# mnhrk15/integrated_path_planning

Measured on AMD Instinct MI355X. Metric: candidate trajectories/sec, higher is better.
Workload: dtype f64; 1 GPU; config4: 256 ego instances/GPU x 2240-candidate lattice (5 s, dt 0.1 s), 20-sample x 30-pedestrian x 51-step fp32 prediction distribution (layout [S][P][T][2]), eps=0; 8 distinct batches rotated (501 MB of obstacle tensors per GPU); instances_per_gpu=256, instances_total=256, rotation_batches=8, plan_calls_in_flight=4

## Files before the change

### integrated_path_planning_amd/csrc/fot_kernels.hip

```cpp
#include <hip/hip_runtime.h>

#include <cstdlib>
#include <cstring>

#include "fot_math.hpp"
#include "fot_kernels.h"

namespace fot {


template <int CTRL, int ROW_MASK>
__device__ __forceinline__ float dpp_f32(float v)
{
    return __int_as_float(__builtin_amdgcn_update_dpp(__float_as_int(v), __float_as_int(v), CTRL, ROW_MASK, 0xf, false));
}

#define FOT_WAVE_REDUCE_F32(NAME, OP)                                                        \
    __device__ __forceinline__ float NAME(float v)                                           \
    {                                                                                        \
        v = OP(v, dpp_f32<0xB1, 0xf>(v));                           \
        v = OP(v, dpp_f32<0x4E, 0xf>(v));                           \
        v = OP(v, dpp_f32<0x141, 0xf>(v));                              \
        v = OP(v, dpp_f32<0x140, 0xf>(v));                                   \
        v = OP(v, dpp_f32<0x142, 0xa>(v));                     \
// ... 376 lines not shown
    if ((int)blockIdx.x < n_inst) {
        if (mixed) {
            const int scen = (imp.h_desc ? imp.h_desc : desc)[blockIdx.x].scen;
            Pp += scen;
            sp_hbm = load_const(sp_table, scen);
        }
        sp = stage_spline(sp_hbm, lds_knots);
    }
    frenet_state_block(Pp, sp, desc, state, n_inst, imp, scan, inst_done, (int)blockIdx.x, gh, all_waves);
}


__device__ __forceinline__ double uniform_f64(double v)
{
    int lo = __builtin_amdgcn_readfirstlane(__double2loint(v));
    int hi = __builtin_amdgcn_readfirstlane(__double2hiint(v));
    asm volatile("" : "+s"(lo), "+s"(hi));
    return __hiloint2double(hi, lo);
}

typedef float f16 __attribute__((ext_vector_type(16)));

template <int OFF>
__device__ __forceinline__ void sload_chunk(f16 &dst, const f2x8 *src)
{
    asm volatile("s_load_dwordx16 %0, %1, %2" : "=s"(dst) : "s"(src), "n"(OFF) : "memory");
}

template <int OFF>
__device__ __forceinline__ void sload_chunk_ahead(f16 &dst, const f2x8 *src, float &ahead)
{
    asm volatile("s_load_dwordx16 %0, %2, %3" : "=s"(dst), "+v"(ahead) : "s"(src), "n"(OFF) : "memory");
}

__device__ __forceinline__ void swait_chunk(f16 &c)
{
    asm volatile("s_waitcnt lgkmcnt(0)" : "+s"(c) : : "memory");
}

typedef float v2f __attribute__((ext_vector_type(2)));

__device__ __forceinline__ float min_sqdist32_f16(const f16 &c, float fx, float fy)
{
    const v2f px = { fx, fx }, py = { fy, fy };
    v2f t[ENT_CHUNK / 2];
#pragma unroll
    for (int j = 0; j < ENT_CHUNK / 2; ++j) {
        const v2f ox = { c[2 * j], c[2 * j + 1] }, oy = { c[8 + 2 * j], c[8 + 2 * j + 1] };
        const v2f dx = px - ox, dy = py - oy;
        t[j] = __builtin_elementwise_fma(dy, dy, dx * dx);
    }
    float m = fminf(fminf(t[0].x, t[0].y), t[1].x);
    m = fminf(fminf(m, t[1].y), t[2].x);
    m = fminf(fminf(m, t[2].y), t[3].x);
    return fminf(m, t[3].y);
}

__device__ __forceinline__ float min_sqdist32_walk(const f2x8 *cp, int n, float &fx, float fy)
{
    float m = INFINITY;
    f16 ca, cb;
    sload_chunk<0>(ca, cp);
    swait_chunk(ca);
    for (int c = 0; c < n; c += 2) {
        sload_chunk_ahead<64>(cb, cp, fx);
        m = fminf(m, min_sqdist32_f16(ca, fx, fy));
        swait_chunk(cb);
        sload_chunk_ahead<128>(ca, cp, fx);
        if (c + 1 < n) m = fminf(m, min_sqdist32_f16(cb, fx, fy));
        swait_chunk(ca);
        cp += 2;
    }
    return m;
}

template <typename T>
__device__ __forceinline__ void st_agent(T *p, T v) { __hip_atomic_store(p, v, __ATOMIC_RELAXED, __HIP_MEMORY_SCOPE_AGENT); }
template <typename T>
__device__ __forceinline__ T ld_agent(const T *p) { return __hip_atomic_load(p, __ATOMIC_RELAXED, __HIP_MEMORY_SCOPE_AGENT); }

struct EvalKernArgs {
    const DevParams *Pp; SplineView sp; const InstDesc *desc; const InstState *state;
    int row_budget, lds_knots, ablate, n_inst, max_tiles;
    const SplineView *sp_table; int mixed;
    const int32_t *tile_cand0;
    const GroupHead *heads;
    const TileStep *wave_rng; const f2 *ent32; const d2 *ent64; const uint8_t *ent_sid;
    double *cand_cost; uint8_t *cand_status; uint16_t *cand_keep;
    TilePart *parts;
    fot_result *out; int32_t *inst_done;
    int32_t *done_flag; int32_t done_seq;
};
constexpr int EVAL_LEAD_PTRS = 7;
__device__ __forceinline__ const EvalKernArgs &eval_kernargs()
{
    return *(const EvalKernArgs *)((const char *)__builtin_amdgcn_kernarg_segment_ptr() + EVAL_LEAD_PTRS * sizeof(void *));
}

template <bool LEAN>
struct FusedSink {
    const DevParams *Pp;
    const InstDesc *Dp;
    uint32_t my_rng;
    float my_thr, my_thr_sure;
    float my_thr_fatal;
    int step_base;
    int step_row;
    int lane_id;
    float thr, thr_fatal;
    const f2x8 *chunks;
    int chunks_per_k;
    uint64_t hit_mask;
    int viol;
    bool hit;
    int c_lo, n_chunks;
    uint32_t pf;
    bool no_warm;

    __device__ __forceinline__ void steps_load(int base)
    {
        const DevParams &P = *Pp;
        const EvalKernArgs &KA = eval_kernargs();
        TileStep st = { 0u, 0.0f, 0.0f, 0u };
        if (Dp->ent_cap != 0 && base + lane_id < P.n_total && !(KA.ablate & 1))
            st = KA.wave_rng[(int64_t)step_row * P.n_total + base + lane_id];
        my_rng = st.rng; my_thr = st.thr; my_thr_sure = st.thr_sure;
        my_thr_fatal = Dp->max_viol == 0 ? st.thr_sure : -1.0f;
        step_base = base;
    }

    __device__ __forceinline__ void row_begin(int k)
    {
        if constexpr (!LEAN)
            if ((k & ~(WAVE - 1)) != step_base) steps_load(k & ~(WAVE - 1));
        const int kl = LEAN ? k : k & (WAVE - 1);
        const uint32_t r = (uint32_t)__builtin_amdgcn_readlane((int)my_rng, kl);
        c_lo = (int)(r >> 16);
        n_chunks = (int)(r & 0xffffu) - c_lo;
        thr = __builtin_bit_cast(float, __builtin_amdgcn_readlane(__builtin_bit_cast(int, my_thr), kl));
        thr_fatal = __builtin_bit_cast(float, __builtin_amdgcn_readlane(__builtin_bit_cast(int, LEAN ? my_thr_sure : my_thr_fatal), kl));
        if (n_chunks > 0 && !no_warm) {
            const f2x8 *row = chunks + (int64_t)k * chunks_per_k + c_lo;
            asm volatile("s_load_dword %0, %1, 0x0\n\t"
                         "s_load_dword %0, %1, 0x40\n\t"
                         "s_load_dword %0, %1, 0x80\n\t"
                         "s_load_dword %0, %1, 0xc0"
                         : "=&s"(pf) : "s"(row) : "memory");
        } else {
            pf = 0;
        }
    }

    __device__ __forceinline__ void row_end(int) { asm volatile("s_waitcnt lgkmcnt(0)" : "+s"(pf) : : "memory"); }

    __device__ __forceinline__ void put(int k, int ci, double px, double py, bool alive)
    {
        put32(k, ci, (float)px, (float)py, alive, [&](double &ex, double &ey) { ex = px; ey = py; });
    }

    template <class GetExact>
    __device__ __forceinline__ void put32(int k, int, float fx_in, float fy, bool alive, const GetExact &get_exact)
    {
        if (n_chunks == 0) return;
        if (!alive || hit) return;
        float fx = fx_in;
        const f2x8 *row = chunks + (int64_t)k * chunks_per_k + c_lo;
        if (LEAN || thr_fatal >= 0.0f) {
            const float m = min_sqdist32_walk(row, n_chunks, fx, fy);
            if (m <= thr_fatal) { hit = true; return; }
            if (!(m <= thr)) return;
        }
        bool sure = false;
        for (int c0 = 0; c0 < n_chunks; c0 += 32) {
            const int nb = n_chunks - c0 < 32 ? n_chunks - c0 : 32;
            const f2x8 *cp = row + c0;
            uint32_t near_bits = 0;
            f16 ca, cb;
            sload_chunk<0>(ca, cp);
            swait_chunk(ca);
            for (int c = 0; c < nb; c += 2) {
                sload_chunk_ahead<64>(cb, cp, fx);
                const float ma = min_sqdist32_f16(ca, fx, fy);
                near_bits = (near_bits << 1) | (uint32_t)(ma <= thr);
                sure |= ma <= thr_fatal;
                swait_chunk(cb);
                sload_chunk_ahead<128>(ca, cp, fx);
                if (c + 1 < nb) {
                    const float mb = min_sqdist32_f16(cb, fx, fy);
                    near_bits = (near_bits << 1) | (uint32_t)(mb <= thr);
                    sure |= mb <= thr_fatal;
                }
                swait_chunk(ca);
                cp += 2;
            }
            if (sure) { hit = true; return; }
            if (near_bits != 0) {
                double px, py;
                get_exact(px, py);
                exact(k, c0, nb, near_bits, px, py, fx, fy);
            }
        }
    }

    __device__ __forceinline__ void exact(int k, int c0, int nb, uint32_t near_bits, double px, double py, float fx,
                                          float fy)
    {
        const DevParams &P = *Pp;
        const InstDesc &D = *Dp;
        px += D.ego.x; py += D.ego.y;
        const double sq_dyn = D.dyn_mode == FOT_DYN_SINGLE ? P.sq_r_dyn : P.sq_r;
        const EvalKernArgs &KA = eval_kernargs();
        const float thr_sure = LEAN ? thr_fatal :
            __builtin_bit_cast(float, __builtin_amdgcn_readlane(__builtin_bit_cast(int, my_thr_sure), k & (WAVE - 1)));
        const d2 *e64 = KA.ent64 + D.ent_off;
        const uint8_t *sid = KA.ent_sid + D.ent_off;
        const int64_t base = ((int64_t)k * chunks_per_k + c_lo) * ENT_CHUNK;
        uint64_t mask_l = 0;
        int viol_l = 0;
        while (near_bits != 0 && !hit) {
            const int hb = 31 - __clz((int)near_bits);
            near_bits &= ~(1u << hb);
            const int64_t e = base + (int64_t)(c0 + nb - 1 - hb) * ENT_CHUNK;
            if constexpr (LEAN)
                exact_chunk_f32first(chunks[e / ENT_CHUNK], e64 + e, sid + e, fx, fy, thr, thr_sure, px, py, P.sq_r, sq_dyn,
                                     0, mask_l, viol_l, hit);
            else
                exact_chunk_f32first(chunks[e / ENT_CHUNK], e64 + e, sid + e, fx, fy, thr, thr_sure, px, py, P.sq_r, sq_dyn,
                                     D.max_viol, hit_mask, viol, hit);
        }
    }

    __device__ __forceinline__ bool collided() const { return hit; }
};

constexpr int EVAL_WG = WAVES_PER_GROUP * WAVE;
extern __shared__ double s_lon[];

constexpr int ROW_FIELDS = 9;
constexpr int LONINFO_DOUBLES = (int)(sizeof(LonInfo) / sizeof(double));
static_assert(sizeof(LonInfo) % sizeof(double) == 0, "LonInfo sits in the double-typed LDS array");
__host__ __device__ constexpr int eval_wave_doubles(int row_budget)
{
    return row_budget * ROW_FIELDS + TILE_MAX_PROFILES * LONINFO_DOUBLES + TILE_MAX_PROFILES / 2;
}
__host__ __device__ constexpr int eval_group_doubles()
{
    return GROUP_ROWS * ROW_FIELDS + (int)(sizeof(GroupHead) / sizeof(double));
}
constexpr int SEG_MAX = 4;
constexpr int SEG_F64 = 4, SEG_I32 = 4;
constexpr int SEG_DOUBLES = (SEG_F64 + SEG_I32 / 2) * WAVE;

struct StagedTab {
    static constexpr bool LOCAL = true;
    int lds_row0;
    int k_max;
    double dt;
#ifdef FOT_TIMELINE
    mutable uint64_t t_rows = 0;
#endif
    __device__ __forceinline__ void load(int k, LonSample &L) const
    {
#ifdef FOT_TIMELINE
        const uint64_t t0 = __builtin_amdgcn_s_memtime();
#endif
        const int kk = k < k_max ? k : k_max;
        const double *r = s_lon + lds_row0 + kk * ROW_FIELDS;
        L.s = 0.0; L.sd = r[0]; L.sdd = r[1]; L.rx = r[2]; L.ry = r[3];
        L.cos_r = r[4]; L.sin_r = r[5]; L.kr = r[6]; L.dkr = r[7]; L.inv_sd = r[8];
        asm volatile("" : "+v"(L.sd), "+v"(L.sdd), "+v"(L.rx), "+v"(L.ry), "+v"(L.cos_r), "+v"(L.sin_r),
                          "+v"(L.kr), "+v"(L.dkr), "+v"(L.inv_sd));
#ifdef FOT_TIMELINE
        t_rows += __builtin_amdgcn_s_memtime() - t0;
#endif
    }
    const LonInfo *info;
    __device__ __forceinline__ double s_at(int k) const
    {
        double s_, u0, u1, u2;
        lon_sample(*info, k, dt, s_, u0, u1, u2);
        return s_;
    }
};

#ifdef FOT_TIMELINE
__device__ uint64_t g_timeline[4 * 16384];
__device__ uint64_t g_shader_clock[2 * 16384];
__device__ uint64_t g_row_wait[16384];
__device__ uint64_t g_phase[4 * 16384];
__shared__ uint64_t s_tl_entry[2];
extern "C" int fot_timeline_read_phase(uint64_t *out, int n_words)
{
    return (int)hipMemcpyFromSymbol(out, HIP_SYMBOL(g_phase), sizeof(uint64_t) * (size_t)n_words);
}
extern "C" int fot_timeline_read_rows(uint64_t *out, int n_words)
{
    return (int)hipMemcpyFromSymbol(out, HIP_SYMBOL(g_row_wait), sizeof(uint64_t) * (size_t)n_words);
}
extern "C" int fot_timeline_read(uint64_t *out, int n_words)
{
    return (int)hipMemcpyFromSymbol(out, HIP_SYMBOL(g_timeline), sizeof(uint64_t) * (size_t)n_words);
}
extern "C" int fot_timeline_read_clock(uint64_t *out, int n_words)
{
    return (int)hipMemcpyFromSymbol(out, HIP_SYMBOL(g_shader_clock), sizeof(uint64_t) * (size_t)n_words);
}
#endif

__device__ __forceinline__ void wave_lds_fence()
{
    __builtin_amdgcn_fence(__ATOMIC_SEQ_CST, "wavefront");
    __builtin_amdgcn_wave_barrier();
}

__device__ __forceinline__ void tile_results(const DevParams &P, const InstDesc &D, const StagedTab &tab, const LonInfo &L,
                                             const double *q, SegState &g, bool hit, bool has_cand, int64_t slot, int cand0,
                                             int lane, TilePart &tp)
{
    int st_final = FOT_ST_DROPPED;
    ScanBest mine = { INFINITY, -1 };
    int my_keep = 0;
    if (has_cand) {
        CandResult r;
        {
            LonInfo Lf = *tab.info;
            Lf.n_t = L.n_t;
            finish_candidate(P, D, Lf, tab, q, g, hit, r);
        }
        st_final = final_status(r.status, r.v_last, r.travel, D.max_stop);
        const EvalKernArgs &KA = eval_kernargs();
        KA.cand_cost[slot] = r.cost;
        KA.cand_status[slot] = (uint8_t)st_final;
        KA.cand_keep[slot] = (uint16_t)r.keep;
        my_keep = r.keep;
        mine = select_entry(st_final, r.cost, cand0 + lane);
    }
    {
        const ScanBest best = wave_argmin(mine);
        tp.cost = best.dist; tp.idx = best.idx;
        tp.keep = __builtin_amdgcn_readfirstlane(__shfl(my_keep, best.idx >= 0 ? best.idx - cand0 : 0, WAVE));
#pragma unroll
        for (int c = 0; c < 8; ++c) tp.cnt[c] = __popcll(__ballot(st_final == c));
    }
}

enum { TILE_WAVE = 0, TILE_SPLIT = 1 };
template <int MODE, bool LEAN>
__device__ __forceinline__ void evaluate_tile(const DevParams *__restrict__ Pp, const InstDesc *__restrict__ desc,
                                              const InstState *__restrict__ state,
                                              const int32_t *__restrict__ tile_cand0, const int32_t *__restrict__ tile_n,
                                              const TileStep *__restrict__ wave_rng, const f2 *__restrict__ ent32,
                                              const EvalKernArgs &a, const SplineView &sp_lds,
                                              double *my_rows, int inst, int tile, int lane, int tl_tag, TilePart &tp,
                                              int sub = 0, int n_sub = 1, double *s_part = nullptr)
{
    constexpr bool SPLIT = MODE == TILE_SPLIT;
    const int seg = SPLIT ? sub : 0, n_seg = SPLIT ? n_sub : 1;
    const DevParams &P = *Pp;
    const InstDesc &D = desc[inst];
    const InstState &S = state[inst];
    const int n_total = P.n_total;
    const int cand0 = tile_cand0[D.shape_off + tile];
    int n = tile_n[D.shape_off + tile];
    int stage_c0 = cand0, stage_c1 = cand0 + n;
    if (n <= 0) return;
    if (!S.c2f_ok || stage_c0 >= S.n_cand) return;
    if (stage_c1 > S.n_cand) stage_c1 = S.n_cand;
    if (cand0 + n > S.n_cand) n = S.n_cand - cand0 > 0 ? S.n_cand - cand0 : 0;
#ifdef FOT_TIMELINE
    const uint64_t t_blk = __builtin_amdgcn_s_memrealtime();
#endif
    LonInfo *s_info = (LonInfo *)(my_rows + a.row_budget * ROW_FIELDS);
    int *s_row0 = (int *)(s_info + TILE_MAX_PROFILES);
    const int slot_lo = decode_candidate(P, D, S.frenet0, stage_c0).lon_slot;
    const int n_stage = decode_candidate(P, D, S.frenet0, stage_c1 - 1).lon_slot - slot_lo + 1;
    const auto lds_fence = [] { if constexpr (MODE != TILE_WAVE) __syncthreads(); else wave_lds_fence(); };
    if constexpr (MODE == TILE_WAVE) wave_lds_fence();
    const int bld_id = (MODE == TILE_WAVE ? 0 : sub * WAVE) + lane, bld_n = (MODE == TILE_WAVE ? 1 : n_sub) * WAVE;
    int total_rows = 0, n_loop = 0;
    for (int p = 0; p < n_stage; ++p) {
        const int r = profile_rows(P, D, slot_lo + p);
        if (bld_id == p) s_row0[p] = total_rows;
        total_rows += r;
    }
    if (bld_id < n_stage) s_info[bld_id] = profile_info(P, D, S.frenet0, slot_lo + bld_id, true);
    lds_fence();
#ifdef FOT_TIMELINE
    const uint64_t t_info = __builtin_amdgcn_s_memrealtime();
#endif
    for (int i = bld_id; i < total_rows; i += bld_n) {
        int p = 0;
        for (int pp = 1; pp < n_stage; ++pp) p = i >= s_row0[pp] ? pp : p;
        const int k = i - s_row0[p];
        const LonInfo Lp = s_info[p];
        LonSample ls;
        double sddd;
        make_lon_sample(sp_lds, Lp, k, P.dt, ls, sddd);
        double *r = my_rows + (int64_t)i * ROW_FIELDS;
        r[0] = ls.sd; r[1] = ls.sdd; r[2] = ls.rx - D.ego.x; r[3] = ls.ry - D.ego.y;
        r[4] = ls.cos_r; r[5] = ls.sin_r; r[6] = ls.kr; r[7] = ls.dkr; r[8] = ls.inv_sd;
    }
    lds_fence();
    constexpr bool SREG = LEAN && SPLIT;
    int ne_min = INT_MAX;
    {
        const int own_lo = decode_candidate(P, D, S.frenet0, cand0).lon_slot - slot_lo;
        const int own_hi = decode_candidate(P, D, S.frenet0, cand0 + n - 1).lon_slot - slot_lo;
        for (int p = own_lo; p <= own_hi; ++p) {
            const int nt = s_info[p].n_t, ne = s_info[p].n_eval;
            n_loop = nt > n_loop ? nt : n_loop; ne_min = ne < ne_min ? ne : ne_min;
        }
        n_loop = __builtin_amdgcn_readfirstlane(n_loop);
        ne_min = __builtin_amdgcn_readfirstlane(ne_min);
    }
    const int seg_len = (n_loop + n_seg - 1) / n_seg;
    const int k0 = SPLIT ? seg * seg_len : 0;
    const int k1 = SPLIT ? (k0 + seg_len < n_loop ? k0 + seg_len : n_loop) : n_loop;

    const int step_base0 = k0 & ~(WAVE - 1);
    TileStep my_step = { 0u, 0.0f, 0.0f, 0u };
    if (D.ent_cap != 0 && step_base0 + lane < n_total && !(a.ablate & 1))
        my_step = wave_rng[(int64_t)(D.tile0 + tile) * n_total + step_base0 + lane];
    const uint32_t my_rng = my_step.rng;
    const float my_thr_fatal = LEAN ? 0.0f : D.max_viol == 0 ? my_step.thr_sure : -1.0f;
#ifdef FOT_TIMELINE
    const uint64_t t_wave = __builtin_amdgcn_s_memrealtime();
    const uint64_t c_wave = __builtin_amdgcn_s_memtime();
    const int tl_wave = D.tile0 + tile;
    uint64_t tl_rows = 0;
    int tl_chunks = (int)(my_rng & 0xffffu) - (int)(my_rng >> 16);
    for (int o = 32; o > 0; o >>= 1) tl_chunks += __shfl_xor(tl_chunks, o);
#endif
    SegState g;
    seg_init(g);
// ... 1082 lines not shown
```

### integrated_path_planning_amd/csrc/fot_math.hpp

```cpp
#pragma once

#include <math.h>
#include "fot_types.h"

namespace fot {


FOT_HD double fast_rcp(double a)
{
#if defined(__HIP_DEVICE_COMPILE__)
    double x = __builtin_amdgcn_rcp(a);
    x = fma(x, fma(-a, x, 1.0), x);
#ifdef FOT_NEWTON2
    x = fma(x, fma(-a, x, 1.0), x);
#endif
    return x;
#else
    return 1.0 / a;
#endif
}

FOT_HD double fast_rsqrt(double a)
{
#if defined(__HIP_DEVICE_COMPILE__)
// ... 266 lines not shown
    L.T = ti.T;
}

FOT_HD void lat_coeffs(const double *fr, double di, const TimeInfo &ti, double *q)
{
#if defined(__clang__)
#pragma clang fp contract(off)
#endif
    const double T = ti.T;
    q[0] = fr[3]; q[1] = fr[4]; q[2] = fr[5] / 2.0;
    const double b0 = di - q[0] - q[1] * T - q[2] * T * T;
    const double b1 = -q[1] - 2.0 * q[2] * T;
    const double b2 = -2.0 * q[2];
    q[3] = b0 * ti.qi[0] + b1 * ti.qi[1] + b2 * ti.qi[2];
    q[4] = b0 * ti.qi[3] + b1 * ti.qi[4] + b2 * ti.qi[5];
    q[5] = b0 * ti.qi[6] + b1 * ti.qi[7] + b2 * ti.qi[8];
}

FOT_HD void lon_eval(const LonInfo &L, double t, double &s, double &sd, double &sdd, double &sddd)
{
    const double t2 = t * t, t3 = t2 * t, t4 = t2 * t2;
    s = L.a0 + L.a1 * t + L.a2 * t2 + L.a3 * t3 + L.a4 * t4;
    sd = L.a1 + 2.0 * L.a2 * t + 3.0 * L.a3 * t2 + 4.0 * L.a4 * t3;
    sdd = 2.0 * L.a2 + 6.0 * L.a3 * t + 12.0 * L.a4 * t2;
    sddd = 6.0 * L.a3 + 24.0 * L.a4 * t;
}

FOT_HD void lat_eval(const double *q, double t, double &d, double &dd, double &ddd, double &dddd)
{
    const double b4 = FOT_FMA(t, q[5], q[4]);
    const double b3 = FOT_FMA(t, b4, q[3]);
    const double b2 = FOT_FMA(t, b3, q[2]);
    const double b1 = FOT_FMA(t, b2, q[1]);
    d = FOT_FMA(t, b1, q[0]);
    const double c4 = FOT_FMA(t, q[5], b4);
    const double c3 = FOT_FMA(t, c4, b3);
    const double c2 = FOT_FMA(t, c3, b2);
    dd = FOT_FMA(t, c2, b1);
    const double e4 = FOT_FMA(t, q[5], c4);
    const double e3 = FOT_FMA(t, e4, c3);
    ddd = 2.0 * FOT_FMA(t, e3, c2);
    dddd = 6.0 * q[3] + t * (24.0 * q[4] + t * (60.0 * q[5]));
}

FOT_HD void lon_sample(const LonInfo &L, int k, double dt, double &s, double &sd, double &sdd, double &sddd)
{
    if (k < L.n_eval) {
        lon_eval(L, (double)k * dt, s, sd, sdd, sddd);
    } else {
        double u0, u1, u2;
        lon_eval(L, (double)(L.n_eval - 1) * dt, s, u0, u1, u2);
        sd = 0.0; sdd = 0.0; sddd = 0.0;
    }
}

FOT_HD void lon_summary(const DevParams &P, LonInfo &L)
{
#if defined(__clang__)
#pragma clang fp contract(off)
#endif
    const double n = (double)L.n_eval, c0 = 6.0 * L.a3, c1 = 24.0 * L.a4 * P.dt;
    const double sum_k = n * (n - 1.0) * 0.5, sum_k2 = (n - 1.0) * n * (2.0 * n - 1.0) / 6.0;
    L.Js = n * c0 * c0 + 2.0 * c0 * c1 * sum_k + c1 * c1 * sum_k2;
    if (L.n_t - 1 < L.n_eval) {
        const double t = (double)(L.n_t - 1) * P.dt, t2 = t * t, t3 = t2 * t;
        L.sd_last = L.a1 + 2.0 * L.a2 * t + 3.0 * L.a3 * t2 + 4.0 * L.a4 * t3;
    } else {
        L.sd_last = 0.0;
    }
}

FOT_HD LonInfo profile_info(const DevParams &P, const InstDesc &D, const double *fr, int slot, bool with_summary)
{
    LonInfo L;
    const int n_grid_lon = P.n_ti * D.n_tv;
    if (slot < n_grid_lon) {
        const int ti = slot / D.n_tv, itv = slot - ti * D.n_tv;
        lon_coeffs(fr, tv_value(P, D, itv), P.ti[ti], L);
        L.n_t = P.ti[ti].n_t;
        L.n_eval = L.n_t;
    } else {
        const TimeInfo &tb = P.brake[slot - n_grid_lon];
        lon_coeffs(fr, 0.0, tb, L);
        L.n_t = P.n_total;
        L.n_eval = tb.n_t;
    }
    L.Js = 0.0; L.sd_last = 0.0;
    if (with_summary) lon_summary(P, L);
    return L;
}

struct LonSlot { int ti, itv; };

FOT_HD LonSlot lon_slot(const DevParams &P, const InstDesc &D, int slot)
{
    LonSlot s;
    const int n_grid_lon = P.n_ti * D.n_tv;
    if (slot < n_grid_lon) { s.ti = slot / D.n_tv; s.itv = slot - s.ti * D.n_tv; }
    else { s.ti = slot - n_grid_lon; s.itv = -1; }
    return s;
}


FOT_HD int profile_rows(const DevParams &P, const InstDesc &D, int slot)
{
    const int n_grid_lon = P.n_ti * D.n_tv;
    if (slot < n_grid_lon) return P.ti[slot / D.n_tv].n_t;
    const int ne = P.brake[slot - n_grid_lon].n_t;
    return ne < P.n_total ? ne + 1 : ne;
}

#ifndef FOT_GROUP_TILES
#define FOT_GROUP_TILES 4
#endif
constexpr int GROUP_TILES = FOT_GROUP_TILES, GROUP_ROWS = 128 * FOT_GROUP_TILES, GROUP_MAX_PROFILES = 4 * FOT_GROUP_TILES;
FOT_HD int tile_row_budget(int n_total)
{
    const int want = 3 * n_total + 8, cap = 176;
    return want < cap ? want : (cap > n_total ? cap : n_total);
}

FOT_HD int tile_extent(const DevParams &P, const InstDesc &D, int cand0, int row_budget)
{
    const int n_grid_lon = P.n_ti * D.n_tv;
    int n = 0, rows = 0, profs = 0, c = cand0;
    while (n < WAVE && c < D.n_cand_max && profs < TILE_MAX_PROFILES) {
        int slot, left;
        if (c < D.n_grid) { slot = c / P.n_di; left = (slot + 1) * P.n_di - c; }
        else { slot = n_grid_lon + (c - D.n_grid); left = 1; }
        const int r = profile_rows(P, D, slot);
        if (profs > 0 && rows + r > row_budget) break;
        rows += r; ++profs;
        const int take = left < WAVE - n ? left : WAVE - n;
        n += take; c += take;
    }
    return n;
}

FOT_HD int count_tiles(const DevParams &P, const InstDesc &D, int row_budget)
{
    int t = 0;
    for (int c = 0; c < D.n_cand_max; ++t) c += tile_extent(P, D, c, row_budget);
    return t;
}


struct LonSample {
    double s, sd, sdd, rx, ry, cos_r, sin_r, kr, dkr;
    double inv_sd;
};

struct CartSample {
    double x, y, cos_t, sin_t, kappa, v, a, omkd;
};

FOT_HD void frenet_to_cart(const LonSample &L, double d, double d_d, double d_dd, CartSample &o)
{
    const double dp = d_d * L.inv_sd;
    const double dpp = (d_dd - dp * L.sdd) * (L.inv_sd * L.inv_sd);
    const double omkd = 1.0 - L.kr * d;
    const double inv_om = fast_rcp(omkd);
    const double hh = dp * dp + omkd * omkd;
    const double inv_h = fast_rsqrt(hh);
    const double h = hh * inv_h;
    const double cos_d = omkd * inv_h, sin_d = dp * inv_h;
    const double tan_d = dp * inv_om;
    const double inv_cos = h * inv_om;
    const double krdp = L.dkr * d + L.kr * dp;
    const double kappa = ((dpp + krdp * tan_d) * omkd * (inv_h * inv_h) + L.kr) * inv_h;
    const double dtp = h * kappa - L.kr;
    o.x = L.rx - L.sin_r * d;
    o.y = L.ry + L.cos_r * d;
    o.cos_t = cos_d * L.cos_r - sin_d * L.sin_r;
    o.sin_t = sin_d * L.cos_r + cos_d * L.sin_r;
    o.kappa = kappa;
    o.v = fabs(L.sd) * h;
    o.a = L.sdd * h + L.sd * L.sd * inv_cos * (dp * dtp - krdp);
    o.omkd = omkd;
}

FOT_HD void load_lon_sample(const double *tab, int k, LonSample &L)
{
    L.s = tab[0 * FOT_MAX_NT + k];   L.sd = tab[1 * FOT_MAX_NT + k];    L.sdd = tab[2 * FOT_MAX_NT + k];
    L.rx = tab[3 * FOT_MAX_NT + k];  L.ry = tab[4 * FOT_MAX_NT + k];
    L.cos_r = tab[5 * FOT_MAX_NT + k]; L.sin_r = tab[6 * FOT_MAX_NT + k];
    L.kr = tab[7 * FOT_MAX_NT + k];  L.dkr = tab[8 * FOT_MAX_NT + k];
    L.inv_sd = tab[9 * FOT_MAX_NT + k];
}

FOT_HD void spline_frame_fast(const SplinePt &p, double &cos_r, double &sin_r, double &kappa, double &dkappa)
{
    const double d = p.dx * p.dx + p.dy * p.dy;
    const double r = fast_rsqrt(d);
    const double r2 = r * r, r3 = r2 * r;
    cos_r = p.dx * r;
    sin_r = p.dy * r;
    const double a = p.dx * p.ddy - p.dy * p.ddx;
    const double b = p.dx * p.dddy - p.dy * p.dddx;
    const double c = p.dx * p.ddx + p.dy * p.ddy;
    kappa = a * r3;
    dkappa = (b - 3.0 * a * c * r2) * r3;
}

FOT_HD void make_lon_sample(const SplineView &sp, const LonInfo &L, int k, double dt, LonSample &o, double &sddd)
{
    lon_sample(L, k, dt, o.s, o.sd, o.sdd, sddd);
    SplinePt p;
    spline_point(sp, o.s, p);
    o.rx = p.x; o.ry = p.y;
    spline_frame_fast(p, o.cos_r, o.sin_r, o.kr, o.dkr);
    o.inv_sd = fabs(o.sd) > 1e-3 ? fast_rcp(o.sd) : 0.0;
}


struct CandResult {
    double cost, v_last, travel;
    int status, keep;
};

struct PathSample {
    double x, y, cos_t, sin_t, kappa, v, a, d;
};

struct LoopConst {
    double dt;
    double lim_speed, lim_accel, lim_curv, lim_lat;
    double road_lim;
    int n_circ_fp;
};

FOT_HD LoopConst loop_const(const DevParams &P, const InstDesc &D)
{
    LoopConst c;
    c.dt = P.dt;
    c.lim_speed = D.lim_speed; c.lim_accel = D.lim_accel; c.lim_curv = D.lim_curv; c.lim_lat = D.lim_lat;
    c.road_lim = P.road_lim;
    c.n_circ_fp = P.has_footprint ? P.n_circ : 0;
    return c;
}

enum : uint32_t {
    CK_NONFINITE = 1u, CK_NANSTEP = 2u, CK_SPEED = 4u, CK_ACCEL = 8u, CK_CURV = 16u, CK_LAT = 32u, CK_ROAD = 64u,
    CK_SINGULAR = 128u, CK_SEEN_NAN = 256u,
    CK_FAILED = CK_NONFINITE | CK_SPEED | CK_ACCEL | CK_CURV | CK_LAT | CK_ROAD | CK_SINGULAR
};

struct CheckAcc {
    uint32_t fl;
    double max_step2;
    PathSample prev;
};

FOT_HD void check_init(CheckAcc &c)
{
    c.fl = 0;
    c.max_step2 = -INFINITY;
    c.prev.x = c.prev.y = c.prev.kappa = c.prev.v = c.prev.a = c.prev.d = 0.0;
    c.prev.cos_t = 1.0; c.prev.sin_t = 0.0;
}

FOT_HD void check_flag(CheckAcc &c, bool cond, uint32_t bit) { c.fl |= cond ? bit : 0u; }

#if defined(__HIP_DEVICE_COMPILE__)
__device__ __attribute__((noinline))
#else
inline
#endif
bool yaw_step_over_cap(double sn, double cs, double lim_curv, double step2)
{
    return fabs(atan2(sn, cs)) > fmax(lim_curv * sqrt(step2), 0.1);
}

#if defined(__HIP_DEVICE_COMPILE__)
#define FOT_KEEP_BRANCH asm volatile("")
#else
#define FOT_KEEP_BRANCH ((void)0)
#endif

FOT_HD void step2_max(double &m, double v)
{
#if defined(__HIP_DEVICE_COMPILE__)
    asm("v_max_f64 %0, %1, %2" : "=v"(m) : "v"(v), "v"(m));
#else
    if (v > m) m = v;
#endif
}

template <class ArcStep>
FOT_HD void check_sample(const LoopConst &C, CheckAcc &c, int k, const PathSample &p, bool has_geo, bool has_d,
                         const ArcStep &arc_step)
{
    check_flag(c, !(isfinite(p.v) && isfinite(p.a) && isfinite(p.kappa)), CK_NONFINITE);
    if (k > 0) {
        const double sx = p.x - c.prev.x, sy = p.y - c.prev.y;
        const double step2 = sum_sq_unfused(sx, sy);
        check_flag(c, isnan(step2), CK_NANSTEP);
        step2_max(c.max_step2, step2);
        check_flag(c, p.v > C.lim_speed, CK_SPEED);
        check_flag(c, fabs(p.a) > C.lim_accel, CK_ACCEL);
        if (p.v > 0.5) {
            check_flag(c, fabs(p.kappa) > C.lim_curv, CK_CURV);
        } else if (has_geo) {
            const double dd = fabs(p.d - c.prev.d);
            const double d_s = arc_step();
            check_flag(c, dd > fmax(1.5 * d_s, 0.02), CK_CURV);
            const double sn = p.sin_t * c.prev.cos_t - p.cos_t * c.prev.sin_t;
            const double cs = p.cos_t * c.prev.cos_t + p.sin_t * c.prev.sin_t;
            if (!(cs > 0.0 && fabs(sn) <= 0.09 * cs)) check_flag(c, yaw_step_over_cap(sn, cs, C.lim_curv, step2), CK_CURV);
        }
        check_flag(c, p.v * p.v * fabs(p.kappa) > C.lim_lat, CK_LAT);
        check_flag(c, has_d && fabs(p.d) > C.road_lim, CK_ROAD);
    }
    c.prev = p;
}

enum : uint32_t { RL_XY = 1u, RL_V = 2u, RL_A = 4u, RL_C = 8u, RL_D = 16u, RL_GEO = 32u };

template <class ArcStep>
FOT_HD void check_sample_ext(const LoopConst &C, CheckAcc &c, int k, const PathSample &p, uint32_t has,
                             const ArcStep &arc_step)
{
    check_flag(c, ((has & RL_V) && !isfinite(p.v)) || ((has & RL_A) && !isfinite(p.a)) ||
                  ((has & RL_C) && !isfinite(p.kappa)), CK_NONFINITE);
    if (k > 0) {
        double step2 = 0.0;
        if (has & RL_XY) {
            step2 = sum_sq_unfused(p.x - c.prev.x, p.y - c.prev.y);
            check_flag(c, isnan(step2), CK_NANSTEP);
            if (step2 > c.max_step2) c.max_step2 = step2;
        }
        check_flag(c, (has & RL_V) && p.v > C.lim_speed, CK_SPEED);
        check_flag(c, (has & RL_A) && fabs(p.a) > C.lim_accel, CK_ACCEL);
        if ((has & RL_V) && (has & RL_C)) {
            if (p.v > 0.5) {
                check_flag(c, fabs(p.kappa) > C.lim_curv, CK_CURV);
            } else if (has & RL_GEO) {
                check_flag(c, fabs(p.d - c.prev.d) > fmax(1.5 * arc_step(), 0.02), CK_CURV);
                const double sn = p.sin_t * c.prev.cos_t - p.cos_t * c.prev.sin_t;
                const double cs = p.cos_t * c.prev.cos_t + p.sin_t * c.prev.sin_t;
                if (!(cs > 0.0 && fabs(sn) <= 0.09 * cs)) check_flag(c, yaw_step_over_cap(sn, cs, C.lim_curv, step2), CK_CURV);
            }
            check_flag(c, p.v * p.v * fabs(p.kappa) > C.lim_lat, CK_LAT);
        }
        check_flag(c, (has & RL_D) && fabs(p.d) > C.road_lim, CK_ROAD);
    }
    c.prev = p;
}

FOT_HD int check_status(const InstDesc &D, const CheckAcc &c, int keep)
{
    if (keep == 0 || (c.fl & CK_NONFINITE) || (!(c.fl & CK_NANSTEP) && sqrt(c.max_step2) > D.step_limit))
        return FOT_ST_DROPPED;
    if (c.fl & CK_SPEED) return FOT_ST_SPEED;
    if (c.fl & CK_ACCEL) return FOT_ST_ACCEL;
    if (c.fl & CK_CURV) return FOT_ST_CURVATURE;
    if (c.fl & CK_LAT) return FOT_ST_LAT_ACCEL;
    if (c.fl & CK_ROAD) return FOT_ST_ROAD;
    return ST_PENDING;
}

FOT_HD void lat_sample(const double *q, int k, int n_eval, double dt, double &d, double &dd, double &ddd, double &dddd)
{
    if (k < n_eval) {
        lat_eval(q, (double)k * dt, d, dd, ddd, dddd);
    } else {
        double u0, u1, u2;
        lat_eval(q, (double)(n_eval - 1) * dt, d, u0, u1, u2);
        dd = 0.0; ddd = 0.0; dddd = 0.0;
    }
}

FOT_HD double lateral_jerk_sum(const double *q, int n_eval, double dt)
{
#if defined(__clang__)
#pragma clang fp contract(off)
#endif
    const double n = (double)n_eval, c0 = 6.0 * q[3], c1 = 24.0 * q[4] * dt, c2 = 60.0 * q[5] * dt * dt;
    const double s1 = n * (n - 1.0) * 0.5, s2 = (n - 1.0) * n * (2.0 * n - 1.0) / 6.0, s3 = s1 * s1;
    const double s4 = (n - 1.0) * n * (2.0 * n - 1.0) * (3.0 * n * n - 3.0 * n - 1.0) / 30.0;
    return c0 * c0 * n + 2.0 * c0 * c1 * s1 + (c1 * c1 + 2.0 * c0 * c2) * s2 + 2.0 * c1 * c2 * s3 + c2 * c2 * s4;
}

struct GlobalTab {
    static constexpr bool LOCAL = false;
    const double *tab;
    FOT_HD void load(int k, LonSample &L) const { load_lon_sample(tab, k, L); }
    FOT_HD double s_at(int k) const { return tab[k]; }
};

struct ComputeTab {
    static constexpr bool LOCAL = false;
    SplineView sp;
    LonInfo L;
    double dt;
    FOT_HD void load(int k, LonSample &o) const
    {
        double sddd;
        if (k < L.n_t) make_lon_sample(sp, L, k, dt, o, sddd);
        else { o.s = o.sd = o.sdd = o.rx = o.ry = o.cos_r = o.sin_r = o.kr = o.dkr = o.inv_sd = 0.0; }
    }
    FOT_HD double s_at(int k) const
    {
        double s_, u0, u1, u2;
        lon_sample(L, k, dt, s_, u0, u1, u2);
        return s_;
    }
};

struct SegState {
    CheckAcc acc;
    double d_last, v_last;
    int first_nan, k_last;
};

FOT_HD void seg_init(SegState &g)
{
    check_init(g.acc);
    g.d_last = 0.0; g.v_last = 0.0;
    g.first_nan = -1; g.k_last = -1;
}

template <bool LEAN = false, bool SREG = true, class Tab, class Sink>
FOT_HD void evaluate_segment(const DevParams &P, const LoopConst &C, const LonInfo &L, const Tab &lon_tab,
                             const double *q, int k0, int k1, Sink &sink, SegState &g, int ne_min = 0)
{
    const int n_t = L.n_t;
    CheckAcc &acc = g.acc;
    if (k0 > 0 && k0 - 1 < n_t) {
        LonSample ls;
        lon_tab.load(k0 - 1, ls);
        double d, d_d, d_dd, d_ddd;
        lat_sample(q, k0 - 1, L.n_eval, C.dt, d, d_d, d_dd, d_ddd);
        CartSample c;
        frenet_to_cart(ls, d, d_d, d_dd, c);
        acc.prev.x = c.x; acc.prev.y = c.y; acc.prev.cos_t = c.cos_t; acc.prev.sin_t = c.sin_t;
        acc.prev.kappa = c.kappa; acc.prev.v = c.v; acc.prev.a = c.a; acc.prev.d = d;
    }
#if defined(__HIP_DEVICE_COMPILE__) && defined(FOT_EVAL_UNROLL)
#pragma unroll FOT_EVAL_UNROLL
#endif
    for (int k = k0; k < k1; ++k) {
      LonSample ls;
      lon_tab.load(k, ls);
      sink.row_begin(k);
      if (k < n_t) {
        double d, d_d, d_dd, d_ddd;
        if constexpr (SREG) {
            const bool may_hold = !(k < ne_min);
            double tk = (double)k;
            if (may_hold) { FOT_KEEP_BRANCH; tk = (double)(k < L.n_eval ? k : L.n_eval - 1); }
            lat_eval(q, tk * C.dt, d, d_d, d_dd, d_ddd);
            if (may_hold) { FOT_KEEP_BRANCH; if (!(k < L.n_eval)) { d_d = 0.0; d_dd = 0.0; d_ddd = 0.0; } }
        } else {
            lat_sample(q, k, L.n_eval, C.dt, d, d_d, d_dd, d_ddd);
        }
        g.d_last = d;
        CartSample c;
        frenet_to_cart(ls, d, d_d, d_dd, c);
        check_flag(acc, isfinite(c.omkd) && c.omkd <= 0.05, CK_SINGULAR);
        if constexpr (SREG) { if (g.first_nan < 0 && isnan(c.x)) g.first_nan = k; }
        else if (!(acc.fl & CK_SEEN_NAN) && isnan(c.x)) { acc.fl |= CK_SEEN_NAN; g.first_nan = k; }
        if (SREG ? g.first_nan < 0 : !(acc.fl & CK_SEEN_NAN)) {
            PathSample ps;
            ps.x = c.x; ps.y = c.y; ps.cos_t = c.cos_t; ps.sin_t = c.sin_t; ps.kappa = c.kappa;
            ps.v = c.v; ps.a = c.a; ps.d = d;
            check_sample(C, acc, k, ps, true, true, [&] { return fabs(lon_tab.s_at(k) - lon_tab.s_at(k - 1)); });
            const bool alive = (acc.fl & CK_FAILED) == 0;
            if constexpr (LEAN) {
                sink.put(k, 0, c.x, c.y, alive);
            } else if (C.n_circ_fp > 0) {
                for (int ci = 0; ci < C.n_circ_fp; ++ci)
                    sink.put(k, ci, c.x + P.circ_off[ci] * c.cos_t, c.y + P.circ_off[ci] * c.sin_t, alive);
            } else {
                sink.put(k, 0, c.x, c.y, alive);
            }
            g.v_last = c.v; g.k_last = k;
        }
      }
      sink.row_end(k);
    }
    if constexpr (SREG) { if (g.first_nan >= 0) acc.fl |= CK_SEEN_NAN; }
}

FOT_HD bool seg_merge(SegState &g, const SegState &n)
{
    g.d_last = n.d_last;
    g.acc.fl |= n.acc.fl & CK_SINGULAR;
    if (g.acc.fl & CK_SEEN_NAN) return false;
    g.acc.fl |= n.acc.fl;
    if (n.acc.max_step2 > g.acc.max_step2) g.acc.max_step2 = n.acc.max_step2;
    if (n.acc.fl & CK_SEEN_NAN) g.first_nan = n.first_nan;
    if (n.k_last >= 0) { g.k_last = n.k_last; g.v_last = n.v_last; }
    return true;
}

template <class Tab>
FOT_HD void finish_candidate(const DevParams &P, const InstDesc &D, const LonInfo &L, const Tab &lon_tab,
                             const double *q, const SegState &g, bool collided, CandResult &out)
{
#if defined(__clang__)
#pragma clang fp contract(off)
#endif
    const int n_t = L.n_t;
    int keep = n_t;
    if (g.acc.fl & CK_SEEN_NAN) keep = g.first_nan >= 2 ? g.first_nan : 0;
    if (g.acc.fl & CK_SINGULAR) keep = 0;

    const double Jd = g.d_last * g.d_last;
    const double dv = D.target_speed - L.sd_last;
    const double Jt = (double)(n_t - 1) * P.dt;
    const double lat = P.k_j * lateral_jerk_sum(q, L.n_eval, P.dt) + P.k_t * Jt + P.k_d * Jd;
    const double lon = P.k_j * L.Js + P.k_t * Jt + P.k_s_dot * (dv * dv);
    out.cost = P.k_lat * lat + P.k_lon * lon;

    int st = check_status(D, g.acc, keep);
    if (st == ST_PENDING && collided) st = FOT_ST_COLLISION;
    out.status = st;
    out.keep = keep;
    out.v_last = g.v_last;
    out.travel = g.k_last >= 0 ? lon_tab.s_at(g.k_last) - lon_tab.s_at(0) : 0.0;
}

template <bool LEAN = false, class Tab, class Sink>
FOT_HD void evaluate_candidate(const DevParams &P, const InstDesc &D, const LoopConst &C, const LonInfo &L,
                               const Tab &lon_tab, const double *q, int n_loop, Sink &sink, CandResult &out)
{
    SegState g;
    seg_init(g);
    evaluate_segment<LEAN>(P, C, L, lon_tab, q, 0, n_loop, sink, g);
    finish_candidate(P, D, L, lon_tab, q, g, sink.collided(), out);
}


struct ObstacleView {
    const void *stat;
    const void *dyn;
    int dtype;
    const uint8_t *nan_track = nullptr;
    FOT_HD d2 at(const void *base, int64_t i) const
    {
        d2 o;
        if (dtype == FOT_F32) { o.x = (double)((const float *)base)[2 * i]; o.y = (double)((const float *)base)[2 * i + 1]; }
        else { o.x = ((const double *)base)[2 * i]; o.y = ((const double *)base)[2 * i + 1]; }
        return o;
    }
    FOT_HD d2 static_at(int j) const { return at(stat, j); }
    FOT_HD d2 dyn_at(int s, int p, int row, int P, int T) const { return at(dyn, ((int64_t)s * P + p) * T + row); }
};

FOT_HD double sum_sq_unfused(double a, double b)
{
#if defined(__clang__)
#pragma clang fp contract(off)
#endif
    const double aa = a * a, bb = b * b;
    return aa + bb;
}

FOT_HD bool within(const d2 &o, double px, double py, double sq)
{
    return sum_sq_unfused(px - o.x, py - o.y) <= sq;
}

template <class Source>
FOT_HD bool collide_candidate(const DevParams &P, const InstDesc &D, const ObstacleView &obs, int keep, const Source &src)
{
    const int n_circ = P.has_footprint ? P.n_circ : 1;
    for (int k = 0; k < keep && D.n_static > 0; ++k)
        for (int ci = 0; ci < n_circ; ++ci) {
            double px, py;
            src.get(k, ci, px, py);
            for (int j = 0; j < D.n_static; ++j)
                if (within(obs.static_at(j), px, py, P.sq_r)) return true;
        }
    if (D.dyn_mode == FOT_DYN_NONE || D.P <= 0 || D.T <= 0) return false;
    const double sq = D.dyn_mode == FOT_DYN_SINGLE ? P.sq_r_dyn : P.sq_r;
    uint64_t hit_mask = 0;
    int viol = 0;
    for (int k = 0; k < keep; ++k) {
        int row = src.tindex(k);
        row = row < 0 ? 0 : (row > D.T - 1 ? D.T - 1 : row);
        for (int ci = 0; ci < n_circ; ++ci) {
            double px, py;
            src.get(k, ci, px, py);
            for (int s = 0; s < D.S; ++s) {
                if ((hit_mask >> s) & 1) continue;
                bool hit = false;
                for (int p = 0; p < D.P; ++p) {
                    if (obs.nan_track && obs.nan_track[s * D.P + p]) continue;
                    if (within(obs.dyn_at(s, p, row, D.P, D.T), px, py, sq)) hit = true;
                }
                if (hit) {
                    hit_mask |= (uint64_t)1 << s;
                    if (++viol > D.max_viol) return true;
                }
            }
        }
    }
    return false;
}


struct Box32 {
    float x0, y0, x1, y1;
};

FOT_HD Box32 box_empty()
{
    Box32 b; b.x0 = INFINITY; b.y0 = INFINITY; b.x1 = -INFINITY; b.y1 = -INFINITY; return b;
}

FOT_HD void box_add(Box32 &b, float x, float y)
{
    b.x0 = fminf(b.x0, x); b.y0 = fminf(b.y0, y); b.x1 = fmaxf(b.x1, x); b.y1 = fmaxf(b.y1, y);
}

FOT_HD void box_merge(Box32 &b, const Box32 &o)
{
    b.x0 = fminf(b.x0, o.x0); b.y0 = fminf(b.y0, o.y0); b.x1 = fmaxf(b.x1, o.x1); b.y1 = fmaxf(b.y1, o.y1);
}

FOT_HD float cull_margin(double max_sq, const Box32 &b)
{
    return sqrtf((float)max_sq) * 1.000001f + 1e-3f
           + 2.4e-7f * (fabsf(b.x0) + fabsf(b.x1) + fabsf(b.y0) + fabsf(b.y1));
}

FOT_HD bool cull_inside(const Box32 &b, float m, float fx, float fy)
{
    return fx >= b.x0 - m && fx <= b.x1 + m && fy >= b.y0 - m && fy <= b.y1 + m;
}

FOT_HD void lateral_extent(const DevParams &P, const double *fr, bool brake, const TimeInfo &ti, int k, int n_eval,
                           double &d0, double &d1)
// ... 709 lines not shown
```

Baseline: 2.920 billion candidates/s.

## Defer limit checks to running maxima and compose headings lazily

```diff
diff --git a/integrated_path_planning_amd/csrc/fot_kernels.hip b/integrated_path_planning_amd/csrc/fot_kernels.hip
--- a/integrated_path_planning_amd/csrc/fot_kernels.hip
+++ b/integrated_path_planning_amd/csrc/fot_kernels.hip
@@ -552,6 +552,8 @@
     }
 
     __device__ __forceinline__ void row_end(int) { asm volatile("s_waitcnt lgkmcnt(0)" : "+s"(pf) : : "memory"); }
+
+    __device__ __forceinline__ bool step_has_points() const { return n_chunks != 0; }
 
     __device__ __forceinline__ void put(int k, int ci, double px, double py, bool alive)
     {
@@ -680,6 +682,12 @@
         double s_, u0, u1, u2;
         lon_sample(*info, k, dt, s_, u0, u1, u2);
         return s_;
+    }
+    __device__ __forceinline__ void frame_at(int k, double &cos_r, double &sin_r) const
+    {
+        const int kk = k < k_max ? k : k_max;
+        const double *r = s_lon + lds_row0 + kk * ROW_FIELDS;
+        cos_r = r[4]; sin_r = r[5];
     }
 };
 
diff --git a/integrated_path_planning_amd/csrc/fot_math.hpp b/integrated_path_planning_amd/csrc/fot_math.hpp
--- a/integrated_path_planning_amd/csrc/fot_math.hpp
+++ b/integrated_path_planning_amd/csrc/fot_math.hpp
@@ -442,8 +442,22 @@
 
 struct CartSample {
     double x, y, cos_t, sin_t, kappa, v, a, omkd;
-};
-
+    double cos_d, sin_d;
+};
+
+FOT_HD void compose_heading(double cos_d, double sin_d, double cos_r, double sin_r, double &cos_t, double &sin_t)
+{
+    cos_t = cos_d * cos_r - sin_d * sin_r;
+    sin_t = sin_d * cos_r + cos_d * sin_r;
+}
+
+FOT_HD void yaw_step_sin_cos(double cos_t, double sin_t, double prev_cos_t, double prev_sin_t, double &sn, double &cs)
+{
+    sn = sin_t * prev_cos_t - cos_t * prev_sin_t;
+    cs = cos_t * prev_cos_t + sin_t * prev_sin_t;
+}
+
+template <bool HEADING = true>
 FOT_HD void frenet_to_cart(const LonSample &L, double d, double d_d, double d_dd, CartSample &o)
 {
     const double dp = d_d * L.inv_sd;
@@ -461,8 +475,8 @@
     const double dtp = h * kappa - L.kr;
     o.x = L.rx - L.sin_r * d;
     o.y = L.ry + L.cos_r * d;
-    o.cos_t = cos_d * L.cos_r - sin_d * L.sin_r;
-    o.sin_t = sin_d * L.cos_r + cos_d * L.sin_r;
+    o.cos_d = cos_d; o.sin_d = sin_d;
+    if constexpr (HEADING) compose_heading(cos_d, sin_d, L.cos_r, L.sin_r, o.cos_t, o.sin_t);
     o.kappa = kappa;
     o.v = fabs(L.sd) * h;
     o.a = L.sdd * h + L.sd * L.sd * inv_cos * (dp * dtp - krdp);
@@ -538,6 +552,7 @@
 struct CheckAcc {
     uint32_t fl;
     double max_step2;
+    double max_v, max_a, max_lat, max_d;
     PathSample prev;
 };
 
@@ -545,6 +560,7 @@
 {
     c.fl = 0;
     c.max_step2 = -INFINITY;
+    c.max_v = c.max_a = c.max_lat = c.max_d = -INFINITY;
     c.prev.x = c.prev.y = c.prev.kappa = c.prev.v = c.prev.a = c.prev.d = 0.0;
     c.prev.cos_t = 1.0; c.prev.sin_t = 0.0;
 }
@@ -576,9 +592,43 @@
 #endif
 }
 
+FOT_HD void abs_max(double &m, double v)
+{
+#if defined(__HIP_DEVICE_COMPILE__)
+    asm("v_max_f64 %0, |%1|, %2" : "=v"(m) : "v"(v), "v"(m));
+#else
+    if (fabs(v) > m) m = fabs(v);
+#endif
+}
+
 template <class ArcStep>
-FOT_HD void check_sample(const LoopConst &C, CheckAcc &c, int k, const PathSample &p, bool has_geo, bool has_d,
-                         const ArcStep &arc_step)
+struct CarriedHeadings {
+    const ArcStep &arc;
+    FOT_HD double arc_step() const { return arc(); }
+    FOT_HD void headings(const PathSample &p, const PathSample &prev, double &ct, double &st, double &pct, double &pst) const
+    {
+        ct = p.cos_t; st = p.sin_t; pct = prev.cos_t; pst = prev.sin_t;
+    }
+};
+template <class Tab, bool HAVE_CUR>
+struct FrameHeadings {
+    const Tab &tab;
+    int k;
+    double cos_c, sin_c;
+    FOT_HD double arc_step() const { return fabs(tab.s_at(k) - tab.s_at(k - 1)); }
+    FOT_HD void headings(const PathSample &p, const PathSample &prev, double &ct, double &st, double &pct, double &pst) const
+    {
+        double pcr, psr;
+        tab.frame_at(k - 1, pcr, psr);
+        if constexpr (HAVE_CUR) { ct = cos_c; st = sin_c; }
+        else compose_heading(p.cos_t, p.sin_t, cos_c, sin_c, ct, st);
+        compose_heading(prev.cos_t, prev.sin_t, pcr, psr, pct, pst);
+    }
+};
+
+template <class Geo>
+FOT_HD void check_sample_geo(const LoopConst &C, CheckAcc &c, int k, const PathSample &p, bool has_geo, bool has_d,
+                             const Geo &geo)
 {
     check_flag(c, !(isfinite(p.v) && isfinite(p.a) && isfinite(p.kappa)), CK_NONFINITE);
     if (k > 0) {
@@ -586,22 +636,43 @@
         const double step2 = sum_sq_unfused(sx, sy);
         check_flag(c, isnan(step2), CK_NANSTEP);
         step2_max(c.max_step2, step2);
-        check_flag(c, p.v > C.lim_speed, CK_SPEED);
-        check_flag(c, fabs(p.a) > C.lim_accel, CK_ACCEL);
-        if (p.v > 0.5) {
-            check_flag(c, fabs(p.kappa) > C.lim_curv, CK_CURV);
-        } else if (has_geo) {
+        step2_max(c.max_v, p.v);
+        abs_max(c.max_a, p.a);
+        step2_max(c.max_lat, p.v * p.v * fabs(p.kappa));
+        if (has_d) abs_max(c.max_d, p.d);
+        const bool fast = p.v > 0.5;
+        check_flag(c, fast && fabs(p.kappa) > C.lim_curv, CK_CURV);
+        if (!fast && has_geo) {
             const double dd = fabs(p.d - c.prev.d);
-            const double d_s = arc_step();
+            const double d_s = geo.arc_step();
             check_flag(c, dd > fmax(1.5 * d_s, 0.02), CK_CURV);
-            const double sn = p.sin_t * c.prev.cos_t - p.cos_t * c.prev.sin_t;
-            const double cs = p.cos_t * c.prev.cos_t + p.sin_t * c.prev.sin_t;
+            double ct, st, pct, pst, sn, cs;
+            geo.headings(p, c.prev, ct, st, pct, pst);
+            yaw_step_sin_cos(ct, st, pct, pst, sn, cs);
             if (!(cs > 0.0 && fabs(sn) <= 0.09 * cs)) check_flag(c, yaw_step_over_cap(sn, cs, C.lim_curv, step2), CK_CURV);
         }
-        check_flag(c, p.v * p.v * fabs(p.kappa) > C.lim_lat, CK_LAT);
-        check_flag(c, has_d && fabs(p.d) > C.road_lim, CK_ROAD);
     }
     c.prev = p;
+}
+
+template <class ArcStep>
+FOT_HD void check_sample(const LoopConst &C, CheckAcc &c, int k, const PathSample &p, bool has_geo, bool has_d,
+                         const ArcStep &arc_step)
+{
+    check_sample_geo(C, c, k, p, has_geo, has_d, CarriedHeadings<ArcStep>{ arc_step });
+}
+
+FOT_HD bool check_over_limit(const LoopConst &C, const CheckAcc &c)
+{
+    return c.max_v > C.lim_speed || c.max_a > C.lim_accel || c.max_lat > C.lim_lat || c.max_d > C.road_lim;
+}
+
+FOT_HD void check_fold(const LoopConst &C, CheckAcc &c)
+{
+    check_flag(c, c.max_v > C.lim_speed, CK_SPEED);
+    check_flag(c, c.max_a > C.lim_accel, CK_ACCEL);
+    check_flag(c, c.max_lat > C.lim_lat, CK_LAT);
+    check_flag(c, c.max_d > C.road_lim, CK_ROAD);
 }
 
 enum : uint32_t { RL_XY = 1u, RL_V = 2u, RL_A = 4u, RL_C = 8u, RL_D = 16u, RL_GEO = 32u };
@@ -676,6 +747,7 @@
     const double *tab;
     FOT_HD void load(int k, LonSample &L) const { load_lon_sample(tab, k, L); }
     FOT_HD double s_at(int k) const { return tab[k]; }
+    FOT_HD void frame_at(int k, double &cos_r, double &sin_r) const { cos_r = tab[5 * FOT_MAX_NT + k]; sin_r = tab[6 * FOT_MAX_NT + k]; }
 };
 
 struct ComputeTab {
@@ -695,6 +767,12 @@
         lon_sample(L, k, dt, s_, u0, u1, u2);
         return s_;
     }
+    FOT_HD void frame_at(int k, double &cos_r, double &sin_r) const
+    {
+        LonSample o;
+        load(k, o);
+        cos_r = o.cos_r; sin_r = o.sin_r;
+    }
 };
 
 struct SegState {
@@ -709,6 +787,11 @@
     g.d_last = 0.0; g.v_last = 0.0;
     g.first_nan = -1; g.k_last = -1;
 }
+
+template <class Sink>
+FOT_HD auto sink_has_points(const Sink &s, int) -> decltype(s.step_has_points()) { return s.step_has_points(); }
+template <class Sink>
+FOT_HD bool sink_has_points(const Sink &, long) { return true; }
 
 template <bool LEAN = false, bool SREG = true, class Tab, class Sink>
 FOT_HD void evaluate_segment(const DevParams &P, const LoopConst &C, const LonInfo &L, const Tab &lon_tab,
@@ -722,8 +805,8 @@
         double d, d_d, d_dd, d_ddd;
         lat_sample(q, k0 - 1, L.n_eval, C.dt, d, d_d, d_dd, d_ddd);
         CartSample c;
-        frenet_to_cart(ls, d, d_d, d_dd, c);
-        acc.prev.x = c.x; acc.prev.y = c.y; acc.prev.cos_t = c.cos_t; acc.prev.sin_t = c.sin_t;
+        frenet_to_cart<false>(ls, d, d_d, d_dd, c);
+        acc.prev.x = c.x; acc.prev.y = c.y; acc.prev.cos_t = c.cos_d; acc.prev.sin_t = c.sin_d;
         acc.prev.kappa = c.kappa; acc.prev.v = c.v; acc.prev.a = c.a; acc.prev.d = d;
     }
 #if defined(__HIP_DEVICE_COMPILE__) && defined(FOT_EVAL_UNROLL)
@@ -746,23 +829,27 @@
         }
         g.d_last = d;
         CartSample c;
-        frenet_to_cart(ls, d, d_d, d_dd, c);
+        frenet_to_cart<!LEAN>(ls, d, d_d, d_dd, c);
         check_flag(acc, isfinite(c.omkd) && c.omkd <= 0.05, CK_SINGULAR);
         if constexpr (SREG) { if (g.first_nan < 0 && isnan(c.x)) g.first_nan = k; }
         else if (!(acc.fl & CK_SEEN_NAN) && isnan(c.x)) { acc.fl |= CK_SEEN_NAN; g.first_nan = k; }
         if (SREG ? g.first_nan < 0 : !(acc.fl & CK_SEEN_NAN)) {
             PathSample ps;
-            ps.x = c.x; ps.y = c.y; ps.cos_t = c.cos_t; ps.sin_t = c.sin_t; ps.kappa = c.kappa;
+            ps.x = c.x; ps.y = c.y; ps.cos_t = c.cos_d; ps.sin_t = c.sin_d; ps.kappa = c.kappa;
             ps.v = c.v; ps.a = c.a; ps.d = d;
-            check_sample(C, acc, k, ps, true, true, [&] { return fabs(lon_tab.s_at(k) - lon_tab.s_at(k - 1)); });
-            const bool alive = (acc.fl & CK_FAILED) == 0;
-            if constexpr (LEAN) {
-                sink.put(k, 0, c.x, c.y, alive);
-            } else if (C.n_circ_fp > 0) {
-                for (int ci = 0; ci < C.n_circ_fp; ++ci)
-                    sink.put(k, ci, c.x + P.circ_off[ci] * c.cos_t, c.y + P.circ_off[ci] * c.sin_t, alive);
-            } else {
-                sink.put(k, 0, c.x, c.y, alive);
+            if constexpr (LEAN) check_sample_geo(C, acc, k, ps, true, true, FrameHeadings<Tab, false>{ lon_tab, k, ls.cos_r, ls.sin_r });
+            else check_sample_geo(C, acc, k, ps, true, true, FrameHeadings<Tab, true>{ lon_tab, k, c.cos_t, c.sin_t });
+            if (sink_has_points(sink, 0)) {
+                FOT_KEEP_BRANCH;
+                const bool alive = (acc.fl & CK_FAILED) == 0 && !check_over_limit(C, acc);
+                if constexpr (LEAN) {
+                    sink.put(k, 0, c.x, c.y, alive);
+                } else if (C.n_circ_fp > 0) {
+                    for (int ci = 0; ci < C.n_circ_fp; ++ci)
+                        sink.put(k, ci, c.x + P.circ_off[ci] * c.cos_t, c.y + P.circ_off[ci] * c.sin_t, alive);
+                } else {
+                    sink.put(k, 0, c.x, c.y, alive);
+                }
             }
             g.v_last = c.v; g.k_last = k;
         }
@@ -770,6 +857,7 @@
       sink.row_end(k);
     }
     if constexpr (SREG) { if (g.first_nan >= 0) acc.fl |= CK_SEEN_NAN; }
+    check_fold(C, acc);
 }
 
 FOT_HD bool seg_merge(SegState &g, const SegState &n)
```

After: 2.982 billion candidates/s (median of 6 runs). 1.02x the previous value.
